# louissmit/VBNN

Measured on NVIDIA B200. Metric: VB-MLP train samples/sec, higher is better.
Workload: dtype bf16

## Files before the change

vbnn_b200/csrc/epilogue_tc.cuh:

```cuda
#pragma once
#include "epilogue.cuh"

namespace vbnn {

constexpr int kStageBytes = 4096;

template <int P>
__device__ __forceinline__ uint32_t stage_off(int row, int piece) {
  if constexpr (P == 8) return (uint32_t)(row * 128 + ((piece ^ (row & 7)) << 4));
  else return (uint32_t)(row * 64 + ((piece ^ ((row >> 1) & 3)) << 4));
}
__device__ __forceinline__ void sts128(uint32_t addr, uint4 v) {
  asm volatile("st.shared.v4.b32 [%0], {%1, %2, %3, %4};" ::"r"(addr), "r"(v.x), "r"(v.y), "r"(v.z), "r"(v.w) : "memory");
}
__device__ __forceinline__ uint4 lds128(uint32_t addr) {
  uint4 v;
  asm volatile("ld.shared.v4.b32 {%0, %1, %2, %3}, [%4];" : "=r"(v.x), "=r"(v.y), "=r"(v.z), "=r"(v.w) : "r"(addr) : "memory");
  return v;
}
__device__ __forceinline__ uint32_t pack_bf16(float a, float b) {
  __nv_bfloat162 t = __floats2bfloat162_rn(a, b);
  return *reinterpret_cast<uint32_t*>(&t);
}
__device__ __forceinline__ uint32_t bf16x2_square(uint32_t w) {
  const __nv_bfloat162 t = *reinterpret_cast<const __nv_bfloat162*>(&w);
  const __nv_bfloat162 r = __hmul2(t, t);
  return *reinterpret_cast<const uint32_t*>(&r);
}
__device__ __forceinline__ float bf16_lo(uint32_t w) { return __uint_as_float(w << 16); }
__device__ __forceinline__ float bf16_hi(uint32_t w) { return __uint_as_float(w & 0xFFFF0000u); }

__device__ __forceinline__ void stage_put_bf16(uint32_t stage, int lane, const uint32_t (&w)[16]) {
#pragma unroll
  for (int pc = 0; pc < 4; ++pc)
    sts128(stage + stage_off<4>(lane, pc), make_uint4(w[4 * pc], w[4 * pc + 1], w[4 * pc + 2], w[4 * pc + 3]));
}
__device__ __forceinline__ void stage_put_f32(uint32_t stage, int lane, const float (&v)[32]) {
#pragma unroll
  for (int pc = 0; pc < 8; ++pc)
    sts128(stage + stage_off<8>(lane, pc),
           make_uint4(__float_as_uint(v[4 * pc]), __float_as_uint(v[4 * pc + 1]), __float_as_uint(v[4 * pc + 2]),
                      __float_as_uint(v[4 * pc + 3])));
}
__device__ __forceinline__ void stage_get_bf16(uint32_t stage, int lane, uint32_t (&w)[16]) {
#pragma unroll
  for (int pc = 0; pc < 4; ++pc) {
    uint4 t = lds128(stage + stage_off<4>(lane, pc));
    w[4 * pc] = t.x; w[4 * pc + 1] = t.y; w[4 * pc + 2] = t.z; w[4 * pc + 3] = t.w;
  }
}
__device__ __forceinline__ void stage_get_f32(uint32_t stage, int lane, float (&v)[32]) {
#pragma unroll
  for (int pc = 0; pc < 8; ++pc) {
    uint4 t = lds128(stage + stage_off<8>(lane, pc));
    v[4 * pc] = __uint_as_float(t.x); v[4 * pc + 1] = __uint_as_float(t.y);
    v[4 * pc + 2] = __uint_as_float(t.z); v[4 * pc + 3] = __uint_as_float(t.w);
  }
}

template <int P>
__device__ __forceinline__ void stage_to_global(uint32_t stage, int lane, char* g, long long ld_bytes, int rows_valid) {
#pragma unroll
  for (int it = 0; it < P; ++it) {
    const int idx = it * 32 + lane, row = idx / P, pc = idx % P;
    const uint4 v = lds128(stage + stage_off<P>(row, pc));
    if (row < rows_valid) __stcs(reinterpret_cast<uint4*>(g + row * ld_bytes + pc * 16), v);
  }
}
template <int P>
__device__ __forceinline__ void global_to_stage(uint32_t stage, int lane, const char* g, long long ld_bytes, int rows_valid) {
  uint4 v[P];
#pragma unroll
  for (int it = 0; it < P; ++it) {
    const int idx = it * 32 + lane, row = idx / P, pc = idx % P;
    v[it] = row < rows_valid ? __ldcs(reinterpret_cast<const uint4*>(g + row * ld_bytes + pc * 16)) : make_uint4(0, 0, 0, 0);
  }
#pragma unroll
  for (int it = 0; it < P; ++it) {
    const int idx = it * 32 + lane, row = idx / P, pc = idx % P;
    sts128(stage + stage_off<P>(row, pc), v[it]);
  }
}

__device__ __forceinline__ void put_tile_bf16(uint32_t stage, int lane, bf16* g, long long ld, int rows_valid,
                                              const uint32_t (&w)[16]) {
  __syncwarp();
  stage_put_bf16(stage, lane, w);
  __syncwarp();
  stage_to_global<4>(stage, lane, reinterpret_cast<char*>(g), ld * 2, rows_valid);
}
__device__ __forceinline__ void put_tile_f32(uint32_t stage, int lane, float* g, long long ld, int rows_valid,
                                             const float (&v)[32]) {
  __syncwarp();
  stage_put_f32(stage, lane, v);
  __syncwarp();
  stage_to_global<8>(stage, lane, reinterpret_cast<char*>(g), ld * 4, rows_valid);
}
__device__ __forceinline__ void get_tile_bf16(uint32_t stage, int lane, const bf16* g, long long ld, int rows_valid,
                                              uint32_t (&w)[16]) {
  __syncwarp();
  global_to_stage<4>(stage, lane, reinterpret_cast<const char*>(g), ld * 2, rows_valid);
  __syncwarp();
  stage_get_bf16(stage, lane, w);
}
__device__ __forceinline__ void get_tile_f32(uint32_t stage, int lane, const float* g, long long ld, int rows_valid,
                                             float (&v)[32]) {
  __syncwarp();
  global_to_stage<8>(stage, lane, reinterpret_cast<const char*>(g), ld * 4, rows_valid);
  __syncwarp();
  stage_get_f32(stage, lane, v);
}

inline bool epi_can_stage(int mode, const EpiParams& p) {
  auto ok_act = [&](const void* ptr, int ld) { return ptr == nullptr || ((ld % 8) == 0 && (reinterpret_cast<uintptr_t>(ptr) % 16) == 0); };
  auto ok_f32 = [&](const void* ptr, int ld) { return ptr == nullptr || ((ld % 4) == 0 && (reinterpret_cast<uintptr_t>(ptr) % 16) == 0); };
  if (p.noise != nullptr) return false;
  if (!ok_f32(p.out_f32, p.ld_f32) || (p.zs_f32 % 4) != 0) return false;
  if (!ok_act(p.out_act, p.ld_act) || !ok_act(p.out_act2, p.ld_act) || !ok_act(p.r_out, p.ld_act) || (p.zs_act % 8) != 0) return false;
  if (!ok_act(p.xprev, p.ld_x) || !ok_act(p.rprev, p.ld_x) || (p.zs_x % 8) != 0) return false;
  if (p.grads_bf16 && (p.ld_g % 8) != 0) return false;
  if (!ok_f32(p.gW, p.ld_g) || !ok_f32(p.gS, p.ld_g)) return false;
  if (!ok_f32(p.aux, p.ld_aux) || (p.zs_aux % 4) != 0) return false;
  if (!ok_act(p.eps16, p.ld_e16) || (p.zs_e16 % 8) != 0) return false;
  if (p.scatter_rows)
    for (int q = 0; q < 8; ++q)
      if (!ok_f32(p.gW_peer[q], p.ld_g) || !ok_f32(p.gS_peer[q], p.ld_g)) return false;
  if (p.bias != nullptr && (reinterpret_cast<uintptr_t>(p.bias) % 16) != 0) return false;
  (void)mode;
  return true;
}

template <int MODE>
__device__ __forceinline__ void epi_chunk_staged(const EpiParams& p, const PhiloxStream& ps0, int z, int row0, int lane,
                                                 int col0, const float (&v1)[32], const float (&v2)[32], uint32_t stage) {
  const int rows_valid = min(32, p.M - row0);
  const int row = row0 + lane;
  if constexpr (MODE == EPI_FWD_LRT2 || MODE == EPI_DX_LRT2) {
    float o[32];
    get_tile_f32(stage, lane, p.aux + z * p.zs_aux + (long long)row0 * p.ld_aux + col0, p.ld_aux, rows_valid, o);
    if constexpr (MODE == EPI_FWD_LRT2) epi_chunk_staged<EPI_FWD_LRT>(p, ps0, z, row0, lane, col0, o, v1, stage);
    else epi_chunk_staged<EPI_DX_LRT>(p, ps0, z, row0, lane, col0, v1, o, stage);
    return;
  }
  if constexpr (MODE == EPI_STORE) {
    put_tile_f32(stage, lane, p.out_f32 + z * p.zs_f32 + (long long)row0 * p.ld_f32 + col0, p.ld_f32, rows_valid, v1);
  } else if constexpr (MODE == EPI_FWD) {
    float y[32];
#pragma unroll
    for (int j = 0; j < 8; ++j) {
      float b[4];
      load_bias4(p.bias, col0 + 4 * j, 4, b);
#pragma unroll
      for (int e = 0; e < 4; ++e) {
        float t = v1[4 * j + e] + b[e];
        y[4 * j + e] = p.relu ? fmaxf(t, 0.f) : t;
      }
    }
    if (p.out_f32)
      put_tile_f32(stage, lane, p.out_f32 + z * p.zs_f32 + (long long)row0 * p.ld_f32 + col0, p.ld_f32, rows_valid, y);
    if (p.out_act) {
      uint32_t w[16];
#pragma unroll
      for (int j = 0; j < 16; ++j) w[j] = pack_bf16(y[2 * j], y[2 * j + 1]);
      put_tile_bf16(stage, lane, (bf16*)p.out_act + z * p.zs_act + (long long)row0 * p.ld_act + col0, p.ld_act, rows_valid, w);
    }
  } else if constexpr (MODE == EPI_FWD_LRT) {
    PhiloxStream ps = ps0;
    ps.sample += (uint32_t)z;
    const uint32_t q = (uint32_t)((p.N + 3) >> 2);
    uint32_t wa[16], w2[16], wr[16];
    float yf[32];
#pragma unroll
    for (int j = 0; j < 8; ++j) {
      float zt[4], b[4];
      philox_normal4(ps, (uint32_t)(row + p.row0) * q + (uint32_t)((col0 >> 2) + j), zt);
      load_bias4(p.bias, col0 + 4 * j, 4, b);
      float ya[4], rr[4];
#pragma unroll
      for (int e = 0; e < 4; ++e) {
        const float v = v2[4 * j + e];
        const float rs = v > 0.f ? rsqrt_fast(v) : 0.f;
        const float y = v1[4 * j + e] + b[e] + (v * rs) * zt[e];
        yf[4 * j + e] = y;
        ya[e] = p.relu ? fmaxf(y, 0.f) : y;
        rr[e] = 0.5f * zt[e] * rs;
      }
      wa[2 * j] = pack_bf16(ya[0], ya[1]); wa[2 * j + 1] = pack_bf16(ya[2], ya[3]);
      wr[2 * j] = pack_bf16(rr[0], rr[1]); wr[2 * j + 1] = pack_bf16(rr[2], rr[3]);
      w2[2 * j] = bf16x2_square(wa[2 * j]); w2[2 * j + 1] = bf16x2_square(wa[2 * j + 1]);
    }
    const long long off = z * p.zs_act + (long long)row0 * p.ld_act + col0;
    if (p.out_f32)
      put_tile_f32(stage, lane, p.out_f32 + z * p.zs_f32 + (long long)row0 * p.ld_f32 + col0, p.ld_f32, rows_valid, yf);
    if (p.out_act) put_tile_bf16(stage, lane, (bf16*)p.out_act + off, p.ld_act, rows_valid, wa);
    if (p.out_act2) put_tile_bf16(stage, lane, (bf16*)p.out_act2 + off, p.ld_act, rows_valid, w2);
    if (p.r_out) put_tile_bf16(stage, lane, (bf16*)p.r_out + off, p.ld_act, rows_valid, wr);
  } else if constexpr (MODE == EPI_DX || MODE == EPI_DX_LRT) {
    const long long xoff = z * p.zs_x + (long long)row0 * p.ld_x + col0;
    uint32_t wx[16];
    const bool need_x = p.xprev != nullptr && (p.mask || MODE == EPI_DX_LRT);
    if (need_x) get_tile_bf16(stage, lane, (const bf16*)p.xprev + xoff, p.ld_x, rows_valid, wx);
    float g[32];
#pragma unroll
    for (int j = 0; j < 16; ++j) {
      const float x0 = need_x ? bf16_lo(wx[j]) : 0.f, x1 = need_x ? bf16_hi(wx[j]) : 0.f;
      float g0 = v1[2 * j], g1 = v1[2 * j + 1];
      if constexpr (MODE == EPI_DX_LRT) { g0 += 2.f * x0 * v2[2 * j]; g1 += 2.f * x1 * v2[2 * j + 1]; }
      if (p.mask) { g0 = x0 > 0.f ? g0 : 0.f; g1 = x1 > 0.f ? g1 : 0.f; }
      g[2 * j] = g0; g[2 * j + 1] = g1;
    }
    if (p.out_f32)
      put_tile_f32(stage, lane, p.out_f32 + z * p.zs_f32 + (long long)row0 * p.ld_f32 + col0, p.ld_f32, rows_valid, g);
    const long long off = z * p.zs_act + (long long)row0 * p.ld_act + col0;
    uint32_t wg[16];
#pragma unroll
    for (int j = 0; j < 16; ++j) wg[j] = pack_bf16(g[2 * j], g[2 * j + 1]);
    if (p.out_act) put_tile_bf16(stage, lane, (bf16*)p.out_act + off, p.ld_act, rows_valid, wg);
    if (p.out_act2 && p.rprev) {
      uint32_t wr[16];
      get_tile_bf16(stage, lane, (const bf16*)p.rprev + xoff, p.ld_x, rows_valid, wr);
#pragma unroll
      for (int j = 0; j < 16; ++j)
        wr[j] = pack_bf16(bf16_lo(wg[j]) * bf16_lo(wr[j]), bf16_hi(wg[j]) * bf16_hi(wr[j]));
      put_tile_bf16(stage, lane, (bf16*)p.out_act2 + off, p.ld_act, rows_valid, wr);
    }
  } else if constexpr (MODE == EPI_DW || MODE == EPI_DW_LRT) {
    const long long goff = (long long)row0 * p.ld_g + col0;
    const bool acc = p.accumulate || z > 0;
    float *gWd, *gSd;
    dw_dest(p, row0, gWd, gSd);
    if (p.grads_bf16) {
      uint32_t w[16];
#pragma unroll
      for (int j = 0; j < 16; ++j) w[j] = pack_bf16(p.scale * v1[2 * j], p.scale * v1[2 * j + 1]);
      put_tile_bf16(stage, lane, reinterpret_cast<bf16*>(gWd) + goff, p.ld_g, rows_valid, w);
      if constexpr (MODE == EPI_DW_LRT) {
        if (p.gS) {
#pragma unroll
          for (int j = 0; j < 16; ++j) w[j] = pack_bf16(v2[2 * j], v2[2 * j + 1]);
          put_tile_bf16(stage, lane, reinterpret_cast<bf16*>(gSd) + goff, p.ld_g, rows_valid, w);
        }
      }
      return;
    }
    float t[32];
    if (acc) {
      get_tile_f32(stage, lane, gWd + goff, p.ld_g, rows_valid, t);
#pragma unroll
      for (int j = 0; j < 32; ++j) t[j] += p.scale * v1[j];
    } else {
#pragma unroll
      for (int j = 0; j < 32; ++j) t[j] = p.scale * v1[j];
    }
    put_tile_f32(stage, lane, gWd + goff, p.ld_g, rows_valid, t);
    if (p.gS) {
      if (acc) get_tile_f32(stage, lane, gSd + goff, p.ld_g, rows_valid, t);
      else {
#pragma unroll
        for (int j = 0; j < 32; ++j) t[j] = 0.f;
      }
// ... 33 lines not shown
```

vbnn_b200/csrc/gemm_tc.cu:

```cuda
#include "gemm.h"
#include "epilogue_tc.cuh"
#include "knobs.h"

#include <cuda.h>
#include <stdlib.h>
#include <string.h>

namespace vbnn {

namespace {

constexpr int BM = 128;
constexpr int BK = 64;
constexpr int UK = 16;
constexpr int EPIW = 8;
constexpr int NTHREADS = (2 + EPIW) * 32;
constexpr int EPI_STAGE_BYTES = EPIW * kStageBytes;
constexpr int SMEM_BUDGET = 227 * 1024 - 2048 - EPI_STAGE_BYTES;

__device__ __forceinline__ uint32_t smem_u32(const void* p) {
  return static_cast<uint32_t>(__cvta_generic_to_shared(p));
}
__device__ __forceinline__ uint32_t cluster_ctarank() {
  uint32_t r;
// ... 186 lines not shown
__device__ __forceinline__ void tmem_st_wait() {
  asm volatile("tcgen05.wait::st.sync.aligned;" ::: "memory");
}

template <bool KMAJOR>
__device__ __forceinline__ uint64_t make_sdesc(uint32_t saddr) {
  constexpr uint64_t lbo = KMAJOR ? 16 : (uint64_t)BK * 128;
  constexpr uint64_t sbo = 1024;
  uint64_t d = 0;
  d |= (uint64_t)((saddr & 0x3FFFFu) >> 4);
  d |= (lbo >> 4) << 16;
  d |= (sbo >> 4) << 32;
  d |= (uint64_t)1 << 46;
  d |= (uint64_t)2 << 61;
  return d;
}
template <bool KMAJOR>
__device__ __forceinline__ constexpr uint32_t kslice_bytes() {
  return KMAJOR ? UK * 2 : UK * 128;
}
template <int BN, int CG, bool AK, bool BKM>
__device__ __forceinline__ constexpr uint32_t make_idesc() {
  return (1u << 4) | (1u << 7) | (1u << 10) | ((AK ? 0u : 1u) << 15) | ((BKM ? 0u : 1u) << 16) |
         ((uint32_t)(BN >> 3) << 17) | ((uint32_t)((BM * CG) >> 4) << 24);
}

struct TcShape {
  int M, N, K, batch;
  int mt, nt, num_kb;
  int gm;
  int staged;
  int clc;
  int zA1, zB1, zA2, zB2;
  int hintA, hintB;
};

__device__ __forceinline__ void decode_tile(const TcShape& sh, int tile, int& mi, int& ni) {
  const int band_tiles = sh.gm * sh.nt;
  const int band = tile / band_tiles;
  const int r = tile - band * band_tiles;
  const int rows = min(sh.gm, sh.mt - band * sh.gm);
  ni = r / rows;
  mi = band * sh.gm + (r - ni * rows);
}

template <int MODE, int BN, int CG>
struct TcCfg {
  static constexpr bool DUAL = epi_is_dual(MODE);
  static constexpr int NACC = DUAL ? 2 : 1;
  static constexpr int A_BYTES = BM * BK * 2;
  static constexpr int B_ROWS = BN / CG;
  static constexpr int B_BYTES = B_ROWS * BK * 2;
  static constexpr int STAGE_BYTES = NACC * (A_BYTES + B_BYTES);
  static constexpr int STAGES_RAW = SMEM_BUDGET / STAGE_BYTES;
  static constexpr int STAGES = STAGES_RAW > 6 ? 6 : STAGES_RAW;
  static constexpr int ACC_COLS = NACC * BN;
  static constexpr int ACC_STAGES = 2 * ACC_COLS <= 512 ? 2 : 1;
  static constexpr bool TACC = epi_z_accumulates(MODE) && !DUAL && BN == 128;
  static constexpr int TMEM_COLS = TACC ? 512 : ACC_STAGES * ACC_COLS;
  static constexpr int SMEM_BYTES = STAGES * STAGE_BYTES + EPI_STAGE_BYTES + 512;
  static_assert(TMEM_COLS == 128 || TMEM_COLS == 256 || TMEM_COLS == 512, "TMEM allocation must be a power of two");
  static_assert(STAGES >= 2, "need at least a double-buffered smem ring");
  static_assert(B_ROWS % 64 == 0, "B tile rows per CTA must be a multiple of 64");
};

template <int CG, bool KMAJOR, int ROWS>
__device__ __forceinline__ void load_operand(const CUtensorMap* tm, uint32_t dst, uint32_t bar,
                                             int mn0, int k0, int z, uint64_t hint) {
  if constexpr (KMAJOR) {
    tma_load_3d<CG>(dst, tm, bar, k0, mn0, z, hint);
  } else {
#pragma unroll
    for (int c = 0; c < ROWS / 64; ++c) tma_load_3d<CG>(dst + c * (BK * 128), tm, bar, mn0 + c * 64, k0, z, hint);
  }
}

template <int MODE, int BN, int CG, bool AK, bool BKM>
__global__ void __launch_bounds__(NTHREADS, 1)
gemm_tc_kernel(const __grid_constant__ CUtensorMap tmA1, const __grid_constant__ CUtensorMap tmB1,
               const __grid_constant__ CUtensorMap tmA2, const __grid_constant__ CUtensorMap tmB2,
               TcShape sh, EpiParams p) {
  using C = TcCfg<MODE, BN, CG>;
  constexpr bool DUAL = C::DUAL;
  constexpr bool ZACC = epi_z_accumulates(MODE);
  constexpr int AS = C::ACC_STAGES;

  extern __shared__ __align__(1024) uint8_t smem_raw[];
  const uint32_t smem_base = smem_u32(smem_raw);
  if ((smem_base & 1023u) != 0) {
    if (threadIdx.x == 0) printf("vbnn gemm_tc: dynamic shared memory base %u is not 1024-byte aligned\n", smem_base);
    __trap();
  }
  const uint32_t epi_stage_base = smem_base + C::STAGES * C::STAGE_BYTES;
  const uint32_t bar_base = epi_stage_base + EPI_STAGE_BYTES;
  auto full_bar = [&](int s) { return bar_base + 8u * s; };
  auto empty_bar = [&](int s) { return bar_base + 8u * (C::STAGES + s); };
  auto tfull_bar = [&](int s) { return bar_base + 8u * (2 * C::STAGES + s); };
  auto tempty_bar = [&](int s) { return bar_base + 8u * (2 * C::STAGES + 2 + s); };
  const uint32_t tmem_slot = bar_base + 8u * (2 * C::STAGES + 4);
  auto clc_resp = [&](int s) { return bar_base + 256u + 16u * s; };
  auto clc_full = [&](int s) { return bar_base + 320u + 8u * s; };
  auto clc_empty = [&](int s) { return bar_base + 336u + 8u * s; };
  constexpr uint32_t kClcConsumers = CG * (1 + EPIW) + 1;

  const int warp = threadIdx.x >> 5, lane = threadIdx.x & 31;
  const int rank = CG == 2 ? (int)cluster_ctarank() : 0;
  const bool leader = rank == 0;

  if (warp == 0 && lane == 0) {
    tma_prefetch_desc(&tmA1);
    tma_prefetch_desc(&tmB1);
    if (DUAL) { tma_prefetch_desc(&tmA2); tma_prefetch_desc(&tmB2); }
    for (int s = 0; s < C::STAGES; ++s) { mbar_init(full_bar(s), 1); mbar_init(empty_bar(s), 1); }
    for (int s = 0; s < 2; ++s) { mbar_init(tfull_bar(s), 1); mbar_init(tempty_bar(s), EPIW * CG); }
    for (int s = 0; s < 2; ++s) { mbar_init(clc_full(s), 1); mbar_init(clc_empty(s), kClcConsumers); }
    fence_barrier_init();
  }
  if (warp == 1) tmem_alloc<CG>(tmem_slot, C::TMEM_COLS);
  tc_fence_before();
  if constexpr (CG == 2) cluster_sync_all(); else __syncthreads();
  tc_fence_after();
  uint32_t tmem_base;
  asm volatile("ld.shared.b32 %0, [%1];" : "=r"(tmem_base) : "r"(tmem_slot));

  const int tiles = sh.mt * sh.nt;
  const int num_work = ZACC ? tiles : tiles * sh.batch;
  const int group = blockIdx.x / CG, num_groups = gridDim.x / CG;
  const bool dyn = sh.clc != 0;
  auto next_work = [&](int w, int& cs, uint32_t& cp, bool whole_warp) -> int {
    if (!dyn) { w += num_groups; return w < num_work ? w : -1; }
    mbar_wait(clc_full(cs), cp);
    const int first = clc_read(clc_resp(cs));
    if (whole_warp) __syncwarp();
    if (!whole_warp || lane == 0) {
      if (CG == 1 || leader) mbar_arrive(clc_empty(cs)); else mbar_arrive_remote(clc_empty(cs), 0);
    }
    if (++cs == 2) { cs = 0; cp ^= 1; }
    return first >= 0 ? first / CG : -1;
  };

  if (warp == 0) {
    if (lane == 0) {
      int stage = 0; uint32_t phase = 0;
      int cs = 0; uint32_t cp = 0;
      int is = 0; uint32_t ip = 0;
      const uint64_t hA = sh.hintA == 1 ? kL2EvictLast : sh.hintA == 2 ? kL2EvictFirst : kL2EvictNormal;
      const uint64_t hB = sh.hintB == 1 ? kL2EvictLast : sh.hintB == 2 ? kL2EvictFirst : kL2EvictNormal;
      for (int w = group; w >= 0 && w < num_work; w = next_work(w, cs, cp, false)) {
        if (dyn && leader) {
          mbar_wait(clc_empty(is), ip ^ 1);
          mbar_expect_tx(clc_full(is), 16);
          if (CG == 2) mbar_expect_tx_remote(clc_full(is), 1, 16);
          clc_try_cancel(clc_resp(is), clc_full(is));
          if (++is == 2) { is = 0; ip ^= 1; }
        }
        const int tile = ZACC ? w : w % tiles;
        const int zb = ZACC ? 0 : w / tiles, zn = ZACC ? sh.batch : 1;
        int mi, ni;
        decode_tile(sh, tile, mi, ni);
        const int m0 = mi * (BM * CG) + rank * BM;
        const int n0 = ni * BN + rank * C::B_ROWS;
        for (int z = zb; z < zb + zn; ++z) {
          for (int kb = 0; kb < sh.num_kb; ++kb) {
            mbar_wait(empty_bar(stage), phase ^ 1);
            if (leader) mbar_expect_tx(full_bar(stage), C::STAGE_BYTES * CG);
            const uint32_t sa = smem_base + stage * C::STAGE_BYTES;
            const uint32_t sb = sa + C::NACC * C::A_BYTES;
            load_operand<CG, AK, BM>(&tmA1, sa, full_bar(stage), m0, kb * BK, z * sh.zA1, hA);
            load_operand<CG, BKM, C::B_ROWS>(&tmB1, sb, full_bar(stage), n0, kb * BK, z * sh.zB1, hB);
            if (DUAL) {
              load_operand<CG, AK, BM>(&tmA2, sa + C::A_BYTES, full_bar(stage), m0, kb * BK, z * sh.zA2, hA);
              load_operand<CG, BKM, C::B_ROWS>(&tmB2, sb + C::B_BYTES, full_bar(stage), n0, kb * BK, z * sh.zB2, hB);
            }
            if (++stage == C::STAGES) { stage = 0; phase ^= 1; }
          }
        }
      }
    }
  } else if (warp == 1) {
    if (lane == 0 && leader) {
      constexpr uint32_t idesc = make_idesc<BN, CG, AK, BKM>();
      int stage = 0; uint32_t phase = 0;
      int as = 0; uint32_t aphase = 0;
      int cs = 0; uint32_t cp = 0;
      for (int w = group; w >= 0 && w < num_work; w = next_work(w, cs, cp, false)) {
        const int zn = ZACC ? sh.batch : 1;
        for (int zi = 0; zi < zn; ++zi) {
          mbar_wait(tempty_bar(as), aphase ^ 1);
          tc_fence_after();
          const uint32_t d1 = tmem_base + as * C::ACC_COLS;
          for (int kb = 0; kb < sh.num_kb; ++kb) {
            mbar_wait(full_bar(stage), phase);
            tc_fence_after();
            const uint32_t sa = smem_base + stage * C::STAGE_BYTES;
            const uint32_t sb = sa + C::NACC * C::A_BYTES;
#pragma unroll
            for (int k = 0; k < BK / UK; ++k) {
              const uint32_t acc = (kb | k) != 0 ? 1u : 0u;
              umma_bf16<CG>(d1, make_sdesc<AK>(sa + k * kslice_bytes<AK>()),
                            make_sdesc<BKM>(sb + k * kslice_bytes<BKM>()), idesc, acc);
              if (DUAL)
                umma_bf16<CG>(d1 + BN, make_sdesc<AK>(sa + C::A_BYTES + k * kslice_bytes<AK>()),
                              make_sdesc<BKM>(sb + C::B_BYTES + k * kslice_bytes<BKM>()), idesc, acc);
            }
            tc_commit<CG>(empty_bar(stage));
            if (++stage == C::STAGES) { stage = 0; phase ^= 1; }
          }
          tc_commit<CG>(tfull_bar(as));
          if (++as == AS) { as = 0; aphase ^= 1; }
        }
      }
    }
  } else {
    const int q = warp & 3;
    const int half = (warp - 2) >> 2;
    const PhiloxStream ps = epi_stream(p);
    const uint32_t my_stage = epi_stage_base + (uint32_t)(warp - 2) * kStageBytes;
    int as = 0; uint32_t aphase = 0;
    int cs = 0; uint32_t cp = 0;
    for (int w = group; w >= 0 && w < num_work; w = next_work(w, cs, cp, true)) {
      const int tile = ZACC ? w : w % tiles;
      const int zb = ZACC ? 0 : w / tiles, zn = ZACC ? sh.batch : 1;
      int mi, ni;
      decode_tile(sh, tile, mi, ni);
      const int m0 = mi * (BM * CG) + rank * BM, n0 = ni * BN;
      const int row = m0 + q * 32 + lane;
      if (C::TACC && zn > 1) {
        const uint32_t lane_base = (uint32_t)(q * 32) << 16;
        const uint32_t tW = tmem_base + lane_base + 256u, tS = tmem_base + lane_base + 384u;
        const uint32_t qn = (uint32_t)((p.N + 3) >> 2);
        for (int z = zb; z < zb + zn; ++z) {
          const bool first = z == zb, last = z + 1 == zb + zn;
          mbar_wait(tfull_bar(as), aphase);
          tc_fence_after();
          const uint32_t tz = tmem_base + lane_base + as * C::ACC_COLS;
          PhiloxStream psz = ps;
          psz.sample += (uint32_t)z;
#pragma unroll 1
          for (int c = half; c < BN / 32; c += EPIW / 4) {
            const int col0 = n0 + c * 32;
            if (col0 >= sh.N) break;
            const int row0 = m0 + q * 32;
            const bool full = sh.staged && col0 + 32 <= sh.N;
            const int rows_valid = min(32, p.M - row0);
            float *gWd, *gSd;
            dw_dest(p, row0, gWd, gSd);
            auto emit = [&](float* dst, float (&a)[32]) {
              const long long goff = (long long)row0 * p.ld_g + col0;
              if (full) {
                if (p.accumulate) {
                  float t[32];
                  get_tile_f32(my_stage, lane, dst + goff, p.ld_g, rows_valid, t);
#pragma unroll
                  for (int j = 0; j < 32; ++j) a[j] += t[j];
                }
                put_tile_f32(my_stage, lane, dst + goff, p.ld_g, rows_valid, a);
              } else if (row < p.M) {
                const bool vec_g = (p.ld_g & 3) == 0;
#pragma unroll
                for (int j = 0; j < 8; ++j) {
                  const int cq = col0 + 4 * j;
                  if (cq >= p.N) break;
                  const int nvalid = min(4, p.N - cq);
                  float* gp = dst + (long long)row * p.ld_g + cq;
                  float w4[4] = {a[4 * j], a[4 * j + 1], a[4 * j + 2], a[4 * j + 3]};
                  if (p.accumulate) { float o[4]; load4<float>(gp, o, nvalid, vec_g); for (int k = 0; k < 4; ++k) w4[k] += o[k]; }
                  store4<float>(gp, w4, nvalid, vec_g);
                }
              }
            };
            float v1[32], acc[32];
            tmem_ld32(tz + c * 32, v1);
// ... 90 lines not shown
            }
          }
          tc_fence_before();
          __syncwarp();
          if (lane == 0) {
            if constexpr (CG == 1) mbar_arrive(tempty_bar(as));
            else mbar_arrive_remote(tempty_bar(as), 0);
          }
          if (++as == AS) { as = 0; aphase ^= 1; }
        }
        if (col0 < sh.N) {
          const int row0 = m0 + q * 32;
          const long long goff = (long long)row0 * p.ld_g + col0;
          float *gWd, *gSd;
          dw_dest(p, row0, gWd, gSd);
          if (sh.staged && col0 + 32 <= sh.N) {
            const int rows_valid = min(32, p.M - row0);
            float t[32];
            if (p.accumulate) {
              get_tile_f32(my_stage, lane, gWd + goff, p.ld_g, rows_valid, t);
#pragma unroll
              for (int j = 0; j < 32; ++j) accW[j] += t[j];
            }
            put_tile_f32(my_stage, lane, gWd + goff, p.ld_g, rows_valid, accW);
            if (p.gS) {
              if (p.accumulate) {
                get_tile_f32(my_stage, lane, gSd + goff, p.ld_g, rows_valid, t);
#pragma unroll
                for (int j = 0; j < 32; ++j) accS[j] += t[j];
              }
              put_tile_f32(my_stage, lane, gSd + goff, p.ld_g, rows_valid, accS);
            }
          } else if (row < p.M) {
            const bool vec_g = (p.ld_g & 3) == 0;
#pragma unroll
            for (int j = 0; j < 8; ++j) {
              const int cq = col0 + 4 * j;
              if (cq >= p.N) break;
              const int nvalid = min(4, p.N - cq);
              float* gw = gWd + (long long)row * p.ld_g + cq;
              float w4[4] = {accW[4 * j], accW[4 * j + 1], accW[4 * j + 2], accW[4 * j + 3]};
              if (p.accumulate) { float o[4]; load4<float>(gw, o, nvalid, vec_g); for (int k = 0; k < 4; ++k) w4[k] += o[k]; }
              store4<float>(gw, w4, nvalid, vec_g);
              if (p.gS) {
                float* gs = gSd + (long long)row * p.ld_g + cq;
                float s4[4] = {accS[4 * j], accS[4 * j + 1], accS[4 * j + 2], accS[4 * j + 3]};
                if (p.accumulate) { float o[4]; load4<float>(gs, o, nvalid, vec_g); for (int k = 0; k < 4; ++k) s4[k] += o[k]; }
                store4<float>(gs, s4, nvalid, vec_g);
              }
            }
          }
        }
      } else {
      for (int z = zb; z < zb + zn; ++z) {
        mbar_wait(tfull_bar(as), aphase);
        tc_fence_after();
        const uint32_t t0 = tmem_base + ((uint32_t)(q * 32) << 16) + as * C::ACC_COLS;
#pragma unroll 1
        for (int c = half; c < BN / 32; c += EPIW / 4) {
          if (n0 + c * 32 >= sh.N) break;
          float v1[32], v2[32];
          tmem_ld32(t0 + c * 32, v1);
          if (DUAL) tmem_ld32(t0 + BN + c * 32, v2);
          tmem_ld_wait();
          if (sh.staged && n0 + c * 32 + 32 <= sh.N) {
            epi_chunk_staged<MODE>(p, ps, z, m0 + q * 32, lane, n0 + c * 32, v1, v2, my_stage);
          } else {
#pragma unroll
            for (int j = 0; j < 8; ++j) {
              epi_quad<MODE, bf16>(p, ps, z, row, n0 + c * 32 + j * 4,
                                   *reinterpret_cast<const float(*)[4]>(&v1[j * 4]),
                                   *reinterpret_cast<const float(*)[4]>(&v2[DUAL ? j * 4 : 0]));
            }
          }
        }
        tc_fence_before();
        __syncwarp();
        if (lane == 0) {
          if constexpr (CG == 1) mbar_arrive(tempty_bar(as));
          else mbar_arrive_remote(tempty_bar(as), 0);
        }
        if (++as == AS) { as = 0; aphase ^= 1; }
      }
      }
    }
  }

  if constexpr (ZACC) { if (p.scatter_rows) __threadfence_system(); }
  tc_fence_before();
  if constexpr (CG == 2) cluster_sync_all(); else __syncthreads();
  if (warp == 1) {
    tc_fence_after();
    tmem_dealloc<CG>(tmem_base, C::TMEM_COLS);
  }
}

typedef CUresult (*PFN_encodeTiled)(CUtensorMap*, CUtensorMapDataType, cuuint32_t, void*,
                                    const cuuint64_t*, const cuuint64_t*, const cuuint32_t*,
                                    const cuuint32_t*, CUtensorMapInterleave, CUtensorMapSwizzle,
                                    CUtensorMapL2promotion, CUtensorMapFloatOOBfill);

PFN_encodeTiled get_encode() {
  static PFN_encodeTiled fn = nullptr;
  if (fn) return fn;
  void* p = nullptr;
  cudaDriverEntryPointQueryResult qr;
  if (cudaGetDriverEntryPoint("cuTensorMapEncodeTiled", &p, cudaEnableDefault, &qr) != cudaSuccess ||
      qr != cudaDriverEntryPointSuccess)
    return nullptr;
  fn = reinterpret_cast<PFN_encodeTiled>(p);
  return fn;
}

int make_tmap(CUtensorMap* tm, const TcOperand& op, int rows_mn, int K, int batch, int box_mn) {
  PFN_encodeTiled enc = get_encode();
  VB_CHECK(enc != nullptr, VBNN_E_CUDA, "cuTensorMapEncodeTiled unavailable (no CUDA driver?)");
  VB_CHECK(op.ptr != nullptr, VBNN_E_INVALID, "gemm_tc: null operand");
  VB_CHECK((op.ld % 8) == 0 && (reinterpret_cast<uintptr_t>(op.ptr) % 16) == 0, VBNN_E_INVALID,
           "gemm_tc: operand rows must be 16-byte aligned (ld=%d)", op.ld);
  VB_CHECK(batch == 1 || (op.zs % 8) == 0, VBNN_E_INVALID, "gemm_tc: batch stride %% 8 != 0");
  cuuint64_t dims[3], strides[2];
  cuuint32_t box[3], estr[3] = {1, 1, 1};
  if (op.kmajor) {
    dims[0] = (cuuint64_t)K; dims[1] = (cuuint64_t)rows_mn;
    box[0] = BK; box[1] = (cuuint32_t)box_mn;
  } else {
    dims[0] = (cuuint64_t)rows_mn; dims[1] = (cuuint64_t)K;
    box[0] = 64; box[1] = BK;
  }
  const bool batched = batch > 1 && op.zs != 0;
  dims[2] = batched ? (cuuint64_t)batch : 1;
  box[2] = 1;
  strides[0] = (cuuint64_t)op.ld * 2;
  strides[1] = batched ? (cuuint64_t)op.zs * 2 : strides[0] * dims[1];
  CUresult r = enc(tm, CU_TENSOR_MAP_DATA_TYPE_BFLOAT16, 3, const_cast<bf16*>(op.ptr), dims, strides,
                   box, estr, CU_TENSOR_MAP_INTERLEAVE_NONE, CU_TENSOR_MAP_SWIZZLE_128B,
                   CU_TENSOR_MAP_L2_PROMOTION_L2_256B, CU_TENSOR_MAP_FLOAT_OOB_FILL_NONE);
  VB_CHECK(r == CUDA_SUCCESS, VBNN_E_CUDA,
// ... 102 lines not shown
  if constexpr (epi_is_dual(MODE)) {
    if (c.cg == 2 && c.bn == 128) return launch_cfg<MODE, 128, 2, AK, BKM>(g, p, st);
  }
  if (c.cg == 2) return launch_cfg<MODE, 256, 2, AK, BKM>(g, p, st);
  if (c.bn == 256 && !epi_is_dual(MODE)) return launch_cfg<MODE, epi_is_dual(MODE) ? 128 : 256, 1, AK, BKM>(g, p, st);
  return launch_cfg<MODE, 128, 1, AK, BKM>(g, p, st);
}

}

void gemm_tc_set_debug(int block_n_override) { g_block_n_override = block_n_override; }

int gemm_tc_launch(int mode, const TcGemmArgs& g, const EpiParams& p, cudaStream_t st,
                   long long* launches) {
  VB_CHECK(g.M > 0 && g.N > 0 && g.K > 0 && g.batch > 0, VBNN_E_INVALID,
           "gemm_tc: empty problem %d x %d x %d (batch %d)", g.M, g.N, g.K, g.batch);
  if (launches) *launches += 1;
  const bool ak = g.A1.kmajor != 0, bk = g.B1.kmajor != 0;
  switch (mode) {
    case EPI_STORE:
      if (ak && bk) return launch_any<EPI_STORE, true, true>(g, p, st);
      if (ak && !bk) return launch_any<EPI_STORE, true, false>(g, p, st);
      if (!ak && bk) return launch_any<EPI_STORE, false, true>(g, p, st);
      return launch_any<EPI_STORE, false, false>(g, p, st);
    case EPI_FWD:
      VB_CHECK(ak && bk, VBNN_E_INVALID, "EPI_FWD expects K-major operands");
      return launch_any<EPI_FWD, true, true>(g, p, st);
    case EPI_FWD_LRT:
      VB_CHECK(ak && bk, VBNN_E_INVALID, "EPI_FWD_LRT expects K-major operands");
      return launch_any<EPI_FWD_LRT, true, true>(g, p, st);
    case EPI_DX:
      VB_CHECK(ak && !bk, VBNN_E_INVALID, "EPI_DX expects K-major A, MN-major B");
      return launch_any<EPI_DX, true, false>(g, p, st);
    case EPI_DX_LRT:
      VB_CHECK(ak && !bk, VBNN_E_INVALID, "EPI_DX_LRT expects K-major A, MN-major B");
      return launch_any<EPI_DX_LRT, true, false>(g, p, st);
    case EPI_FWD_LRT2:
      VB_CHECK(ak && bk && p.aux, VBNN_E_INVALID, "EPI_FWD_LRT2 expects K-major operands and the mean product");
      return launch_any<EPI_FWD_LRT2, true, true>(g, p, st);
    case EPI_DX_LRT2:
      VB_CHECK(ak && !bk && p.aux, VBNN_E_INVALID, "EPI_DX_LRT2 expects K-major A, MN-major B and the H s2 product");
      return launch_any<EPI_DX_LRT2, true, false>(g, p, st);
    case EPI_DW:
      VB_CHECK(!ak && !bk, VBNN_E_INVALID, "EPI_DW expects MN-major operands");
      return launch_any<EPI_DW, false, false>(g, p, st);
    case EPI_DW_LRT:
      VB_CHECK(!ak && !bk, VBNN_E_INVALID, "EPI_DW_LRT expects MN-major operands");
      return launch_any<EPI_DW_LRT, false, false>(g, p, st);
  }
  set_error("gemm_tc_launch: bad mode %d", mode);
  return VBNN_E_INVALID;
}

}
```

Measured before the change: 1.455 million.

## Prefetch epilogue operands ahead and release TMEM accumulator early

Adds a per-mode look-ahead for the DX_LRT epilogues. For DX_LRT, the xprev and rprev tiles for the next chunk are loaded into registers early, and the later columns get L2 prefetches. For DX_LRT2, the aux f32 tile is double-buffered with cp.async into an extra shared buffer, which takes shared memory away from the mainloop stage ring. The TMEM accumulator is also released right after the last tmem load instead of after the epilogue math. The aim is to hide global load latency in the epilogue and let the MMA warp start the next tile sooner. An optional compile-time timing instrumentation is included.

Result: no change. 1.457 million, median of 6 (+0.1%).

```diff
diff --git a/vbnn_b200/csrc/epilogue_tc.cuh b/vbnn_b200/csrc/epilogue_tc.cuh
--- a/vbnn_b200/csrc/epilogue_tc.cuh
+++ b/vbnn_b200/csrc/epilogue_tc.cuh
@@ -4,6 +4,56 @@
 namespace vbnn {
 
 constexpr int kStageBytes = 4096;
+
+enum EpiPhase : int {
+  EPT_TILES,
+  EPT_WAIT,
+  EPT_TMEM,
+  EPT_LOAD,
+  EPT_MATH,
+  EPT_STORE,
+  EPT_MMA_TILES,
+  EPT_MMA_WAIT,
+  EPT_CYCLES,
+  EPT_NS,
+  EPT_N
+};
+#ifdef VBNN_EPI_TIMING
+__device__ unsigned long long g_epi_timing[9][EPT_N];
+struct EpiTimer {
+  int mode;
+  bool on;
+  long long t, t0;
+  unsigned long long ns0;
+  __device__ __forceinline__ EpiTimer(int mode_, bool on_) : mode(mode_), on(on_) {
+    t = t0 = clock64();
+    asm volatile("mov.u64 %0, %%globaltimer;" : "=l"(ns0));
+  }
+  __device__ __forceinline__ void reset() { t = clock64(); }
+  __device__ __forceinline__ void mark(int phase) {
+    const long long now = clock64();
+    if (on) atomicAdd(&g_epi_timing[mode][phase], (unsigned long long)(now - t));
+    t = now;
+  }
+  __device__ __forceinline__ void count(int phase) { if (on) atomicAdd(&g_epi_timing[mode][phase], 1ull); }
+  __device__ __forceinline__ void finish() {
+    unsigned long long ns;
+    asm volatile("mov.u64 %0, %%globaltimer;" : "=l"(ns));
+    if (on) {
+      atomicAdd(&g_epi_timing[mode][EPT_CYCLES], (unsigned long long)(clock64() - t0));
+      atomicAdd(&g_epi_timing[mode][EPT_NS], ns - ns0);
+    }
+  }
+};
+#else
+struct EpiTimer {
+  __device__ __forceinline__ EpiTimer(int, bool) {}
+  __device__ __forceinline__ void reset() {}
+  __device__ __forceinline__ void mark(int) {}
+  __device__ __forceinline__ void count(int) {}
+  __device__ __forceinline__ void finish() {}
+};
+#endif
 
 template <int P>
 __device__ __forceinline__ uint32_t stage_off(int row, int piece) {
@@ -68,19 +118,40 @@
   }
 }
 template <int P>
-__device__ __forceinline__ void global_to_stage(uint32_t stage, int lane, const char* g, long long ld_bytes, int rows_valid) {
-  uint4 v[P];
+__device__ __forceinline__ void global_pieces(uint4 (&v)[P], int lane, const char* g, long long ld_bytes, int rows_valid) {
 #pragma unroll
   for (int it = 0; it < P; ++it) {
     const int idx = it * 32 + lane, row = idx / P, pc = idx % P;
     v[it] = row < rows_valid ? __ldcs(reinterpret_cast<const uint4*>(g + row * ld_bytes + pc * 16)) : make_uint4(0, 0, 0, 0);
   }
+}
+template <int P>
+__device__ __forceinline__ void pieces_to_stage(uint32_t stage, int lane, const uint4 (&v)[P]) {
 #pragma unroll
   for (int it = 0; it < P; ++it) {
     const int idx = it * 32 + lane, row = idx / P, pc = idx % P;
     sts128(stage + stage_off<P>(row, pc), v[it]);
   }
 }
+template <int P>
+__device__ __forceinline__ void global_to_stage(uint32_t stage, int lane, const char* g, long long ld_bytes, int rows_valid) {
+  uint4 v[P];
+  global_pieces<P>(v, lane, g, ld_bytes, rows_valid);
+  pieces_to_stage<P>(stage, lane, v);
+}
+template <int P>
+__device__ __forceinline__ void global_to_stage_async(uint32_t stage, int lane, const char* g, long long ld_bytes, int rows_valid,
+                                                      const void* base) {
+#pragma unroll
+  for (int it = 0; it < P; ++it) {
+    const int idx = it * 32 + lane, row = idx / P, pc = idx % P;
+    const char* src = row < rows_valid ? g + row * ld_bytes + pc * 16 : static_cast<const char*>(base);
+    asm volatile("cp.async.cg.shared.global [%0], [%1], 16, %2;" ::"r"(stage + stage_off<P>(row, pc)), "l"(src),
+                 "r"(row < rows_valid ? 16 : 0) : "memory");
+  }
+  asm volatile("cp.async.commit_group;" ::: "memory");
+}
+__device__ __forceinline__ void cp_async_wait() { asm volatile("cp.async.wait_group 0;" ::: "memory"); }
 
 __device__ __forceinline__ void put_tile_bf16(uint32_t stage, int lane, bf16* g, long long ld, int rows_valid,
                                               const uint32_t (&w)[16]) {
@@ -130,16 +201,121 @@
   return true;
 }
 
+template <int MODE> struct EpiAhead {
+  __device__ __forceinline__ void start_tile(const EpiParams&, int, int, int, int, int, int) {}
+  __device__ __forceinline__ void fetch(const EpiParams&, int, int, int, int) {}
+};
+template <> struct EpiAhead<EPI_DX_LRT> {
+  uint4 x[4], r[4];
+  __device__ __forceinline__ void fetch(const EpiParams& p, int z, int row0, int col0, int lane) {
+    const int rows_valid = min(32, p.M - row0);
+    const long long xoff = z * p.zs_x + (long long)row0 * p.ld_x + col0;
+    const uint4 zero = make_uint4(0, 0, 0, 0);
+    if (p.xprev) global_pieces<4>(x, lane, reinterpret_cast<const char*>((const bf16*)p.xprev + xoff), p.ld_x * 2LL, rows_valid);
+    else x[0] = x[1] = x[2] = x[3] = zero;
+    if (p.out_act2 && p.rprev)
+      global_pieces<4>(r, lane, reinterpret_cast<const char*>((const bf16*)p.rprev + xoff), p.ld_x * 2LL, rows_valid);
+    else r[0] = r[1] = r[2] = r[3] = zero;
+  }
+  __device__ __forceinline__ void start_tile(const EpiParams& p, int z, int row0, int col0, int step, int col_end, int lane) {
+    fetch(p, z, row0, col0, lane);
+    if (row0 + lane >= p.M) return;
+    const long long xrow = z * p.zs_x + (long long)(row0 + lane) * p.ld_x;
+    for (int c = col0 + step; c + 32 <= col_end; c += step) {
+      if (p.xprev) asm volatile("prefetch.global.L2 [%0];" ::"l"((const bf16*)p.xprev + xrow + c));
+      if (p.out_act2 && p.rprev) asm volatile("prefetch.global.L2 [%0];" ::"l"((const bf16*)p.rprev + xrow + c));
+    }
+  }
+};
+struct EpiAheadAux {
+  uint32_t buf;
+  __device__ __forceinline__ void fetch(const EpiParams& p, int z, int row0, int col0, int lane) {
+    global_to_stage_async<8>(buf, lane, reinterpret_cast<const char*>(p.aux + z * p.zs_aux + (long long)row0 * p.ld_aux + col0),
+                             p.ld_aux * 4LL, min(32, p.M - row0), p.aux);
+  }
+  __device__ __forceinline__ void start_tile(const EpiParams& p, int z, int row0, int col0, int, int, int lane) {
+    fetch(p, z, row0, col0, lane);
+  }
+  __device__ __forceinline__ void take(int lane, float (&o)[32]) {
+    cp_async_wait();
+    __syncwarp();
+    stage_get_f32(buf, lane, o);
+    __syncwarp();
+  }
+};
+template <> struct EpiAhead<EPI_DX_LRT2> : EpiAheadAux {};
+
+__device__ __forceinline__ void epi_dx_lrt_staged(const EpiParams& p, int z, int row0, int lane, int col0,
+                                                  const float (&v1)[32], const float (&v2)[32], uint32_t stage, EpiTimer& tm) {
+  const int rows_valid = min(32, p.M - row0);
+  uint32_t wx[16], wr[16];
+  __syncwarp();
+  stage_get_bf16(stage, lane, wx);
+  stage_get_bf16(stage + 2048, lane, wr);
+  tm.mark(EPT_LOAD);
+  float g[32];
+#pragma unroll
+  for (int j = 0; j < 16; ++j) {
+    const float x0 = bf16_lo(wx[j]), x1 = bf16_hi(wx[j]);
+    float g0 = v1[2 * j], g1 = v1[2 * j + 1];
+    g0 += 2.f * x0 * v2[2 * j]; g1 += 2.f * x1 * v2[2 * j + 1];
+    if (p.mask) { g0 = x0 > 0.f ? g0 : 0.f; g1 = x1 > 0.f ? g1 : 0.f; }
+    g[2 * j] = g0; g[2 * j + 1] = g1;
+  }
+  uint32_t wg[16];
+#pragma unroll
+  for (int j = 0; j < 16; ++j) wg[j] = pack_bf16(g[2 * j], g[2 * j + 1]);
+  const bool h = p.out_act2 && p.rprev;
+  if (h) {
+#pragma unroll
+    for (int j = 0; j < 16; ++j)
+      wr[j] = pack_bf16(bf16_lo(wg[j]) * bf16_lo(wr[j]), bf16_hi(wg[j]) * bf16_hi(wr[j]));
+  }
+  tm.mark(EPT_MATH);
+  if (p.out_f32)
+    put_tile_f32(stage, lane, p.out_f32 + z * p.zs_f32 + (long long)row0 * p.ld_f32 + col0, p.ld_f32, rows_valid, g);
+  const long long off = z * p.zs_act + (long long)row0 * p.ld_act + col0;
+  __syncwarp();
+  if (p.out_act) stage_put_bf16(stage, lane, wg);
+  if (h) stage_put_bf16(stage + 2048, lane, wr);
+  __syncwarp();
+  if (p.out_act) stage_to_global<4>(stage, lane, reinterpret_cast<char*>((bf16*)p.out_act + off), p.ld_act * 2LL, rows_valid);
+  if (h) stage_to_global<4>(stage + 2048, lane, reinterpret_cast<char*>((bf16*)p.out_act2 + off), p.ld_act * 2LL, rows_valid);
+  tm.mark(EPT_STORE);
+}
+
 template <int MODE>
 __device__ __forceinline__ void epi_chunk_staged(const EpiParams& p, const PhiloxStream& ps0, int z, int row0, int lane,
-                                                 int col0, const float (&v1)[32], const float (&v2)[32], uint32_t stage) {
+                                                 int col0, const float (&v1)[32], const float (&v2)[32], uint32_t stage,
+                                                 EpiTimer& tm, EpiAhead<MODE>& ahead, int next_col) {
   const int rows_valid = min(32, p.M - row0);
   const int row = row0 + lane;
-  if constexpr (MODE == EPI_FWD_LRT2 || MODE == EPI_DX_LRT2) {
+  if constexpr (MODE == EPI_FWD_LRT2) {
     float o[32];
     get_tile_f32(stage, lane, p.aux + z * p.zs_aux + (long long)row0 * p.ld_aux + col0, p.ld_aux, rows_valid, o);
-    if constexpr (MODE == EPI_FWD_LRT2) epi_chunk_staged<EPI_FWD_LRT>(p, ps0, z, row0, lane, col0, o, v1, stage);
-    else epi_chunk_staged<EPI_DX_LRT>(p, ps0, z, row0, lane, col0, v1, o, stage);
+    tm.mark(EPT_LOAD);
+    EpiAhead<EPI_FWD_LRT> none;
+    epi_chunk_staged<EPI_FWD_LRT>(p, ps0, z, row0, lane, col0, o, v1, stage, tm, none, -1);
+    return;
+  }
+  if constexpr (MODE == EPI_DX_LRT2) {
+    float o[32];
+    ahead.take(lane, o);
+    if (next_col >= 0) ahead.fetch(p, z, row0, next_col, lane);
+    EpiAhead<EPI_DX_LRT> xr;
+    xr.fetch(p, z, row0, col0, lane);
+    __syncwarp();
+    pieces_to_stage<4>(stage, lane, xr.x);
+    pieces_to_stage<4>(stage + 2048, lane, xr.r);
+    epi_dx_lrt_staged(p, z, row0, lane, col0, v1, o, stage, tm);
+    return;
+  }
+  if constexpr (MODE == EPI_DX_LRT) {
+    __syncwarp();
+    pieces_to_stage<4>(stage, lane, ahead.x);
+    pieces_to_stage<4>(stage + 2048, lane, ahead.r);
+    if (next_col >= 0) ahead.fetch(p, z, row0, next_col, lane);
+    epi_dx_lrt_staged(p, z, row0, lane, col0, v1, v2, stage, tm);
     return;
   }
   if constexpr (MODE == EPI_STORE) {
@@ -189,23 +365,24 @@
       wr[2 * j] = pack_bf16(rr[0], rr[1]); wr[2 * j + 1] = pack_bf16(rr[2], rr[3]);
       w2[2 * j] = bf16x2_square(wa[2 * j]); w2[2 * j + 1] = bf16x2_square(wa[2 * j + 1]);
     }
+    tm.mark(EPT_MATH);
     const long long off = z * p.zs_act + (long long)row0 * p.ld_act + col0;
     if (p.out_f32)
       put_tile_f32(stage, lane, p.out_f32 + z * p.zs_f32 + (long long)row0 * p.ld_f32 + col0, p.ld_f32, rows_valid, yf);
     if (p.out_act) put_tile_bf16(stage, lane, (bf16*)p.out_act + off, p.ld_act, rows_valid, wa);
     if (p.out_act2) put_tile_bf16(stage, lane, (bf16*)p.out_act2 + off, p.ld_act, rows_valid, w2);
     if (p.r_out) put_tile_bf16(stage, lane, (bf16*)p.r_out + off, p.ld_act, rows_valid, wr);
-  } else if constexpr (MODE == EPI_DX || MODE == EPI_DX_LRT) {
+    tm.mark(EPT_STORE);
+  } else if constexpr (MODE == EPI_DX) {
     const long long xoff = z * p.zs_x + (long long)row0 * p.ld_x + col0;
     uint32_t wx[16];
-    const bool need_x = p.xprev != nullptr && (p.mask || MODE == EPI_DX_LRT);
+    const bool need_x = p.xprev != nullptr && p.mask;
     if (need_x) get_tile_bf16(stage, lane, (const bf16*)p.xprev + xoff, p.ld_x, rows_valid, wx);
     float g[32];
 #pragma unroll
     for (int j = 0; j < 16; ++j) {
       const float x0 = need_x ? bf16_lo(wx[j]) : 0.f, x1 = need_x ? bf16_hi(wx[j]) : 0.f;
       float g0 = v1[2 * j], g1 = v1[2 * j + 1];
-      if constexpr (MODE == EPI_DX_LRT) { g0 += 2.f * x0 * v2[2 * j]; g1 += 2.f * x1 * v2[2 * j + 1]; }
       if (p.mask) { g0 = x0 > 0.f ? g0 : 0.f; g1 = x1 > 0.f ? g1 : 0.f; }
       g[2 * j] = g0; g[2 * j + 1] = g1;
     }
diff --git a/vbnn_b200/csrc/gemm_tc.cu b/vbnn_b200/csrc/gemm_tc.cu
--- a/vbnn_b200/csrc/gemm_tc.cu
+++ b/vbnn_b200/csrc/gemm_tc.cu
@@ -262,13 +262,14 @@
   static constexpr int B_ROWS = BN / CG;
   static constexpr int B_BYTES = B_ROWS * BK * 2;
   static constexpr int STAGE_BYTES = NACC * (A_BYTES + B_BYTES);
-  static constexpr int STAGES_RAW = SMEM_BUDGET / STAGE_BYTES;
+  static constexpr int AUX_BYTES = MODE == EPI_DX_LRT2 ? EPI_STAGE_BYTES : 0;
+  static constexpr int STAGES_RAW = (SMEM_BUDGET - AUX_BYTES) / STAGE_BYTES;
   static constexpr int STAGES = STAGES_RAW > 6 ? 6 : STAGES_RAW;
   static constexpr int ACC_COLS = NACC * BN;
   static constexpr int ACC_STAGES = 2 * ACC_COLS <= 512 ? 2 : 1;
   static constexpr bool TACC = epi_z_accumulates(MODE) && !DUAL && BN == 128;
   static constexpr int TMEM_COLS = TACC ? 512 : ACC_STAGES * ACC_COLS;
-  static constexpr int SMEM_BYTES = STAGES * STAGE_BYTES + EPI_STAGE_BYTES + 512;
+  static constexpr int SMEM_BYTES = STAGES * STAGE_BYTES + EPI_STAGE_BYTES + AUX_BYTES + 512;
   static_assert(TMEM_COLS == 128 || TMEM_COLS == 256 || TMEM_COLS == 512, "TMEM allocation must be a power of two");
   static_assert(STAGES >= 2, "need at least a double-buffered smem ring");
   static_assert(B_ROWS % 64 == 0, "B tile rows per CTA must be a multiple of 64");
@@ -302,7 +303,8 @@
     __trap();
   }
   const uint32_t epi_stage_base = smem_base + C::STAGES * C::STAGE_BYTES;
-  const uint32_t bar_base = epi_stage_base + EPI_STAGE_BYTES;
+  const uint32_t aux_base = epi_stage_base + EPI_STAGE_BYTES;
+  const uint32_t bar_base = aux_base + C::AUX_BYTES;
   auto full_bar = [&](int s) { return bar_base + 8u * s; };
   auto empty_bar = [&](int s) { return bar_base + 8u * (C::STAGES + s); };
   auto tfull_bar = [&](int s) { return bar_base + 8u * (2 * C::STAGES + s); };
@@ -393,10 +395,14 @@
       int stage = 0; uint32_t phase = 0;
       int as = 0; uint32_t aphase = 0;
       int cs = 0; uint32_t cp = 0;
+      EpiTimer tm(MODE, true);
       for (int w = group; w >= 0 && w < num_work; w = next_work(w, cs, cp, false)) {
         const int zn = ZACC ? sh.batch : 1;
         for (int zi = 0; zi < zn; ++zi) {
+          tm.reset();
           mbar_wait(tempty_bar(as), aphase ^ 1);
+          tm.mark(EPT_MMA_WAIT);
+          tm.count(EPT_MMA_TILES);
           tc_fence_after();
           const uint32_t d1 = tmem_base + as * C::ACC_COLS;
           for (int kb = 0; kb < sh.num_kb; ++kb) {
@@ -428,6 +434,9 @@
     const uint32_t my_stage = epi_stage_base + (uint32_t)(warp - 2) * kStageBytes;
     int as = 0; uint32_t aphase = 0;
     int cs = 0; uint32_t cp = 0;
+    EpiTimer tm(MODE, lane == 0);
+    EpiAhead<MODE> ahead;
+    if constexpr (C::AUX_BYTES > 0) ahead.buf = aux_base + (uint32_t)(warp - 2) * kStageBytes;
     for (int w = group; w >= 0 && w < num_work; w = next_work(w, cs, cp, true)) {
       const int tile = ZACC ? w : w % tiles;
       const int zb = ZACC ? 0 : w / tiles, zn = ZACC ? sh.batch : 1;
@@ -624,10 +633,25 @@
           }
         }
       } else {
+      auto staged_chunk = [&](int c) { return sh.staged && c < BN / 32 && n0 + c * 32 + 32 <= sh.N; };
       for (int z = zb; z < zb + zn; ++z) {
+        if (staged_chunk(half))
+          ahead.start_tile(p, z, m0 + q * 32, n0 + half * 32, 32 * (EPIW / 4), min(n0 + BN, sh.N), lane);
         mbar_wait(tfull_bar(as), aphase);
+        tm.mark(EPT_WAIT);
+        tm.count(EPT_TILES);
         tc_fence_after();
         const uint32_t t0 = tmem_base + ((uint32_t)(q * 32) << 16) + as * C::ACC_COLS;
+        bool freed = false;
+        auto free_acc = [&]() {
+          tc_fence_before();
+          __syncwarp();
+          if (lane == 0) {
+            if constexpr (CG == 1) mbar_arrive(tempty_bar(as));
+            else mbar_arrive_remote(tempty_bar(as), 0);
+          }
+          freed = true;
+        };
 #pragma unroll 1
         for (int c = half; c < BN / 32; c += EPIW / 4) {
           if (n0 + c * 32 >= sh.N) break;
@@ -635,8 +659,12 @@
           tmem_ld32(t0 + c * 32, v1);
           if (DUAL) tmem_ld32(t0 + BN + c * 32, v2);
           tmem_ld_wait();
-          if (sh.staged && n0 + c * 32 + 32 <= sh.N) {
-            epi_chunk_staged<MODE>(p, ps, z, m0 + q * 32, lane, n0 + c * 32, v1, v2, my_stage);
+          if (c + EPIW / 4 >= BN / 32 || n0 + (c + EPIW / 4) * 32 >= sh.N) free_acc();
+          tm.mark(EPT_TMEM);
+          if (staged_chunk(c)) {
+            const int cn = c + EPIW / 4;
+            epi_chunk_staged<MODE>(p, ps, z, m0 + q * 32, lane, n0 + c * 32, v1, v2, my_stage, tm, ahead,
+                                   staged_chunk(cn) ? n0 + cn * 32 : -1);
           } else {
 #pragma unroll
             for (int j = 0; j < 8; ++j) {
@@ -645,17 +673,14 @@
                                    *reinterpret_cast<const float(*)[4]>(&v2[DUAL ? j * 4 : 0]));
             }
           }
+          tm.mark(EPT_STORE);
         }
-        tc_fence_before();
-        __syncwarp();
-        if (lane == 0) {
-          if constexpr (CG == 1) mbar_arrive(tempty_bar(as));
-          else mbar_arrive_remote(tempty_bar(as), 0);
-        }
+        if (!freed) free_acc();
         if (++as == AS) { as = 0; aphase ^= 1; }
       }
       }
     }
+    tm.finish();
   }
 
   if constexpr (ZACC) { if (p.scatter_rows) __threadfence_system(); }
@@ -864,4 +889,14 @@
   return VBNN_E_INVALID;
 }
 
-}
+#ifdef VBNN_EPI_TIMING
+extern "C" int vbnn_epi_timing_read(unsigned long long* out) {
+  VB_CUDA(cudaDeviceSynchronize());
+  VB_CUDA(cudaMemcpyFromSymbol(out, g_epi_timing, sizeof(g_epi_timing)));
+  static const unsigned long long zero[9][EPT_N] = {};
+  VB_CUDA(cudaMemcpyToSymbol(g_epi_timing, zero, sizeof(zero)));
+  return VBNN_OK;
+}
+#endif
+
+}
```
